# alehdaghi/vq-vae-2-pytorch

Measured on AMD Instinct MI355X. Metric: images/sec VQ-VAE-2 256px train step, higher is better.
Workload: dtype f32; 1 GPU; configs[1]: 256x256 FFHQ-shaped synthetic, default two-level VQ-VAE-2, batch 32/GPU; global_batch=32, image=256, n_embed=512, parallelism=dp1

## Files before the change

include/vq2.h:

```cpp
#ifndef VQ2_H
#define VQ2_H

#include <stddef.h>
#include <stdint.h>

#ifdef __cplusplus
extern "C" {
#endif

#define VQ2_OK 0
#define VQ2_ERR_INVALID 1
#define VQ2_ERR_UNSUPPORTED 2
#define VQ2_ERR_WORKSPACE 3
#define VQ2_ERR_LAUNCH 4

typedef void *vq2_stream_t;

#define VQ2_API_VERSION 6

int vq2_version(void);
const char *vq2_last_error(void);

int vq2_prof_enable(int level);
int vq2_prof_report(char *buf, size_t cap);

typedef struct vq2_conv_desc {
    int32_t N, H, W, Ci;
    int32_t Co;
    int32_t KH, KW, stride, pad;
    int32_t transposed;
    int32_t ldx, ldy;
    int32_t Cir, Cor;
} vq2_conv_desc;

#define VQ2_RELU_IN 1
#define VQ2_RELU_OUT 2

#define VQ2_PACK_FWD 0
#define VQ2_PACK_DGRAD 1
int vq2_pack_weight(const vq2_conv_desc *d, int which, const float *w, float *packed, vq2_stream_t stream);

typedef struct vq2_pack_job {
    const float *w;
    float *packed;
    int64_t offset;
    int64_t numel;
    int32_t Or, Ir, Op, Ip, KH, KW, mode, reserved;
} vq2_pack_job;
int vq2_pack_job_init(const vq2_conv_desc *d, int which, const float *w, float *packed, vq2_pack_job *job);
int vq2_pack_weights_batched(const vq2_pack_job *jobs_dev, int32_t njobs, int64_t total, vq2_stream_t stream);

int vq2_conv_fwd(const vq2_conv_desc *d, int flags, const float *x, const float *wp, const float *bias,
                 const float *residual, int32_t ldres, float *y, vq2_stream_t stream);

int vq2_resblock_supported(int32_t C, int32_t Cm);
int vq2_resblock_fwd(int32_t N, int32_t H, int32_t W, int32_t C, int32_t Cm, int flags, const float *x, int32_t ldx,
                     const float *w1p, const float *b1, const float *w2p, const float *b2, float *r, int32_t ldr,
                     float *y, int32_t ldy, vq2_stream_t stream);

size_t vq2_resblock_w2_workspace_bytes(int32_t N, int32_t H, int32_t W, int32_t C, int32_t Cm);
int vq2_resblock_bwd_data(int32_t N, int32_t H, int32_t W, int32_t C, int32_t Cm, const float *g, int32_t ldg,
                          const float *r, int32_t ldr, const float *x, int32_t ldx, const float *w2d, const float *w1d,
                          float *dh, int32_t lddh, float *dx, int32_t lddx, void *w2_ws, vq2_stream_t stream);

int vq2_conv_dgrad(const vq2_conv_desc *d, const float *dy, const float *wp, const float *mask, int32_t ldmask,
                   const float *residual, int32_t ldres, float *dx, int32_t lddx, vq2_stream_t stream);
#define VQ2_MASK_AFTER_RESIDUAL 4
int vq2_conv_dgrad_ex(const vq2_conv_desc *d, int flags, const float *dy, const float *wp, const float *mask,
                      int32_t ldmask, const float *residual, int32_t ldres, float *dx, int32_t lddx,
                      vq2_stream_t stream);

size_t vq2_conv_wgrad_workspace_bytes(const vq2_conv_desc *d);
int vq2_conv_wgrad(const vq2_conv_desc *d, int flags, const float *x, const float *dy, float *dw, float *db, void *ws,
                   size_t ws_bytes, vq2_stream_t stream);

typedef struct vq2_wgrad_job {
    const float *ws;
    float *dw;
    const float *bias_ws;
    float *db;
    int64_t unit_offset;
    int32_t O, I, Or, Ir, taps, S, n_units_w, n_units_b;
    int32_t swapped;
    int32_t bias_splits;
} vq2_wgrad_job;
int vq2_conv_wgrad_partial(const vq2_conv_desc *d, int flags, const float *x, const float *dy, float *db, void *ws,
                           size_t ws_bytes, vq2_stream_t stream);
int vq2_wgrad_job_init(const vq2_conv_desc *d, const void *ws, float *dw, float *db, vq2_wgrad_job *job);
int vq2_wgrad_reduce_batched(const vq2_wgrad_job *jobs_dev, int32_t njobs, int64_t total_units, vq2_stream_t stream);
int vq2_resblock_w2_job_init(int32_t N, int32_t H, int32_t W, int32_t C, int32_t Cm, const void *ws, float *dw, float *db,
                             vq2_wgrad_job *job);

size_t vq2_colsum_workspace_bytes(int64_t rows, int32_t C);
int vq2_colsum(const float *dy, int64_t rows, int32_t C, int32_t ld, float *db, void *ws, size_t ws_bytes,
               vq2_stream_t stream);

// ... 80 lines not shown
```

vq-vae-2-pytorch_amd/_lib.py:

```python
import ctypes as C
import os

_HERE = os.path.dirname(os.path.abspath(__file__))
LIB_PATH = os.environ.get("VQ2_LIB") or os.path.join(_HERE, "libvq2.so")

c_f32p = C.c_void_p
c_stream = C.c_void_p


class ConvDesc(C.Structure):
    _fields_ = [(n, C.c_int32) for n in
                ("N", "H", "W", "Ci", "Co", "KH", "KW", "stride", "pad", "transposed", "ldx", "ldy", "Cir", "Cor")]


class PackJob(C.Structure):
    _fields_ = [("w", C.c_void_p), ("packed", C.c_void_p), ("offset", C.c_int64), ("numel", C.c_int64)] + \
               [(n, C.c_int32) for n in ("Or", "Ir", "Op", "Ip", "KH", "KW", "mode", "reserved")]


class WgradJob(C.Structure):
    _fields_ = [("ws", C.c_void_p), ("dw", C.c_void_p), ("bias_ws", C.c_void_p), ("db", C.c_void_p),
                ("unit_offset", C.c_int64)] + \
               [(n, C.c_int32) for n in ("O", "I", "Or", "Ir", "taps", "S", "n_units_w", "n_units_b", "swapped", "bias_splits")]

# ... 7 lines not shown
    lib = C.CDLL(LIB_PATH)
    P, I32, I64, SZ, F, D = C.c_void_p, C.c_int32, C.c_int64, C.c_size_t, C.c_float, C.c_double
    DP = C.POINTER(ConvDesc)
    sig = {
        "vq2_version": (C.c_int, []),
        "vq2_last_error": (C.c_char_p, []),
        "vq2_prof_enable": (C.c_int, [C.c_int]),
        "vq2_prof_report": (C.c_int, [C.c_char_p, SZ]),
        "vq2_pack_weight": (C.c_int, [DP, C.c_int, P, P, P]),
        "vq2_pack_job_init": (C.c_int, [DP, C.c_int, P, P, C.POINTER(PackJob)]),
        "vq2_pack_weights_batched": (C.c_int, [P, I32, I64, P]),
        "vq2_conv_fwd": (C.c_int, [DP, C.c_int, P, P, P, P, I32, P, P]),
        "vq2_conv_dgrad": (C.c_int, [DP, P, P, P, I32, P, I32, P, I32, P]),
        "vq2_conv_dgrad_ex": (C.c_int, [DP, C.c_int, P, P, P, I32, P, I32, P, I32, P]),
        "vq2_conv_wgrad_workspace_bytes": (SZ, [DP]),
        "vq2_conv_wgrad": (C.c_int, [DP, C.c_int, P, P, P, P, P, SZ, P]),
        "vq2_conv_wgrad_partial": (C.c_int, [DP, C.c_int, P, P, P, P, SZ, P]),
        "vq2_wgrad_job_init": (C.c_int, [DP, P, P, P, C.POINTER(WgradJob)]),
        "vq2_wgrad_reduce_batched": (C.c_int, [P, I32, I64, P]),
        "vq2_colsum_workspace_bytes": (SZ, [I64, I32]),
        "vq2_colsum": (C.c_int, [P, I64, I32, I32, P, P, SZ, P]),
        "vq2_nchw_to_nhwc": (C.c_int, [P, P, I32, I32, I32, I32, I32, P]),
        "vq2_nhwc_to_nchw": (C.c_int, [P, P, I32, I32, I32, I32, I32, P]),
        "vq2_u8_to_nhwc4": (C.c_int, [P, C.c_int, I32, I32, I32, I32, I32, I32, I32, I32, P, P, P]),
        "vq2_nhwc_to_u8": (C.c_int, [P, I32, I32, I32, I32, I32, C.POINTER(F), C.POINTER(F), P, C.c_int, I32, I32, I64, I32,
                                     I32, I64, P]),
        "vq2_sse_workspace_bytes": (SZ, [I32, I32, I32, I32]),
        "vq2_sse_per_image": (C.c_int, [P, P, I32, I32, I32, I32, P, P, SZ, P]),
        "vq2_index_hist": (C.c_int, [P, I64, I32, P, P, P]),
        "vq2_eval_accumulate": (C.c_int, [P, I32, I64, P, P, P]),
        "vq2_relu_bwd": (C.c_int, [P, I32, P, I32, P, I32, I64, I32, P]),
        "vq2_resblock_supported": (C.c_int, [I32, I32]),
        "vq2_resblock_bwd_data": (C.c_int, [I32, I32, I32, I32, I32, P, I32, P, I32, P, I32, P, P, P, I32, P, I32, P, P]),
        "vq2_resblock_w2_workspace_bytes": (SZ, [I32, I32, I32, I32, I32]),
        "vq2_resblock_w2_job_init": (C.c_int, [I32, I32, I32, I32, I32, P, P, P, C.POINTER(WgradJob)]),
        "vq2_resblock_fwd": (C.c_int, [I32, I32, I32, I32, I32, C.c_int, P, I32, P, P, P, P, P, I32, P, I32, P]),
        "vq2_slice_copy": (C.c_int, [P, I32, P, I32, I64, I32, C.c_int, P]),
        "vq2_vq_prepare": (C.c_int, [P, P, P, I32, I32, P]),
        "vq2_vq_fwd_workspace_floats": (SZ, [I64, I32, I32]),
        "vq2_vq_fwd": (C.c_int, [P, I32, P, P, P, I64, I32, I32, P, P, I32, P, P]),
        "vq2_vq_stats_workspace_bytes": (SZ, [I64, I32, I32]),
        "vq2_vq_stats": (C.c_int, [P, I32, P, I64, I32, I32, P, P, P, SZ, P]),
        "vq2_vq_loss": (C.c_int, [P, I64, I32, P, P]),
        "vq2_vq_bwd": (C.c_int, [P, I32, P, P, I32, P, P, I64, I32, I32, P, I32, P]),
        "vq2_vq_ema_update": (C.c_int, [P, P, P, P, P, I32, I32, D, D, P, P]),
        "vq2_vq_ema_update_prepare": (C.c_int, [P, P, P, P, P, I32, I32, D, D, P, P, P, P]),
        "vq2_vq_gather": (C.c_int, [P, P, I64, I32, I32, P, I32, P]),
        "vq2_instnorm_stats": (C.c_int, [P, I32, I32, I64, I32, D, P, P, P]),
        "vq2_adain_fwd": (C.c_int, [P, I32, P, P, P, I32, I64, I32, C.c_int, P, I32, P]),
        "vq2_adain_bwd": (C.c_int, [P, I32, P, I32, P, I32, P, P, P, I32, I64, I32, P, P, I32, P]),
        "vq2_mse_workspace_bytes": (SZ, [I64]),
        "vq2_mse_fwd_bwd": (C.c_int, [P, P, I64, I64, P, P, P, P, SZ, P]),
        "vq2_stage1_loss": (C.c_int, [P, P, I64, I64, P, F, P, P, P, P, SZ, P]),
        "vq2_adam_step": (C.c_int, [P, P, P, P, I64, D, D, D, D, I32, D, P]),
        "vq2_axpby": (C.c_int, [P, P, F, P, I64, P]),
        "vq2_scale": (C.c_int, [P, P, F, P, I64, P]),
        "vq2_comm_unique_id": (C.c_int, [P]),
        "vq2_comm_init": (C.c_int, [P, I32, I32]),
        "vq2_comm_world": (C.c_int, []),
        "vq2_comm_rank": (C.c_int, []),
        "vq2_comm_allreduce_sum": (C.c_int, [P, I64, P]),
        "vq2_comm_broadcast": (C.c_int, [P, I64, I32, P]),
        "vq2_comm_destroy": (C.c_int, []),
        "vq2_debug_mfma_peak": (C.c_int, [P, I32, I32, P]),
        "vq2_debug_mfma_peak16": (C.c_int, [P, I32, I32, P]),
    }
# ... 26 lines not shown
```

vq-vae-2-pytorch_amd/csrc/vq2_resblock.hip:

```cpp
#include "vq2_common.h"
#include "vq2_rbwino.h"

namespace vq2 {

typedef unsigned int u32x4 __attribute__((ext_vector_type(4)));

namespace rb {
constexpr unsigned RSRC_FLAGS = 0x00020000;
constexpr int OOB = 0x7F000000;
constexpr int TH = 8, TW = 16;
constexpr int PW = TW + 2, PH = TH + 2;
constexpr int NPATCH = PW * PH;
constexpr int CS = 16;
constexpr int LDK = CS + 4;
constexpr int CM = 32;
constexpr int CC = 128;
constexpr int A_F4 = NPATCH * CS / 4;
constexpr int B_F4 = 9 * CM * CS / 4;
constexpr int A_FLOATS = ((A_F4 + 255) / 256) * 64 * LDK;
constexpr int B_FLOATS = ((B_F4 + 255) / 256) * 64 * LDK;
constexpr int LDR = CM + 4;
constexpr size_t LDS_BYTES = (size_t)2 * (A_FLOATS + B_FLOATS) * sizeof(float);
static_assert(2 * LDS_BYTES <= 160 * 1024, "two workgroups per CU");
static_assert(128 * LDR <= 2 * (A_FLOATS + B_FLOATS), "stage-2 aliases fit in the stage-1 buffers");
}

struct ResFwdParams {
    const float *x;
    const float *w1;
    const float *b1;
    const float *w2;
    const float *b2;
    float *r;
    float *y;
// ... 233 lines not shown
        __builtin_amdgcn_raw_buffer_store_b32(__float_as_uint(v), ry, yoff[r] + (NJ - 1) * 128, 0, 0);
    }
}


namespace rbb {
using namespace rb;
constexpr int SA = 32;
constexpr int LDA = SA + 4;
constexpr int PROWS = 192;
constexpr int GA_FLOATS = PROWS * LDA;
constexpr int WA_FLOATS = CM * LDA;
constexpr int WB_FLOATS = CC * LDA;
constexpr size_t LDS_BYTES = (size_t)(2 * GA_FLOATS + 2 * WA_FLOATS) * sizeof(float);
constexpr int WR_FLOATS = 16 * 64 + 32;
constexpr size_t LDS_BYTES_W2 = LDS_BYTES + (size_t)4 * WR_FLOATS * sizeof(float);
static_assert(GA_FLOATS + 2 * WB_FLOATS <= 2 * GA_FLOATS + 2 * WA_FLOATS, "phase-B buffers alias the phase-A ones");
}

struct ResBwdParams {
    const float *g;
    const float *r;
    const float *x;
    const float *w2d;
    const float *w1d;
    float *dh;
    float *dx;
    float *w2_slab;
    float *b2_slab;
    int N, H, W, ldg, ldr, ldx, lddh, lddx;
    int tiles_x, tiles_y;
};

template <bool SAME_LD>
__global__ __launch_bounds__(256, 2) void resblock_bwd_data_kernel(const ResBwdParams P) {
    using namespace rbb;
    extern __shared__ __attribute__((aligned(16))) float smem[];
    float *Ga = smem;
    float *Wa = smem + 2 * GA_FLOATS;
    float *Dh = smem;
    float *Wb = smem + GA_FLOATS;

    const int tid = threadIdx.x, lane = tid & 63, wq = tid >> 6;
    const int l31 = lane & 31, fk = 4 * (lane >> 5), rowq = 4 * (lane >> 5);
    const int tiles = P.tiles_x * P.tiles_y;
    const int vid = xcd_remap(blockIdx.x, gridDim.x);
    const int n = vid / tiles;
    const int t = vid - n * tiles;
    const int tyi = t / P.tiles_x;
    const int y0 = tyi * TH, x0 = (t - tyi * P.tiles_x) * TW;
    const int npix = P.N * P.H * P.W;
    const __amdgpu_buffer_rsrc_t rg = __builtin_amdgcn_make_buffer_rsrc(const_cast<float *>(P.g), 0, npix * P.ldg * 4, RSRC_FLAGS);
    const __amdgpu_buffer_rsrc_t rr = __builtin_amdgcn_make_buffer_rsrc(const_cast<float *>(P.r), 0, npix * P.ldr * 4, RSRC_FLAGS);
    const __amdgpu_buffer_rsrc_t rx = __builtin_amdgcn_make_buffer_rsrc(const_cast<float *>(P.x), 0, npix * P.ldx * 4, RSRC_FLAGS);
    const __amdgpu_buffer_rsrc_t rw2 = __builtin_amdgcn_make_buffer_rsrc(const_cast<float *>(P.w2d), 0, CM * CC * 4, RSRC_FLAGS);
    const __amdgpu_buffer_rsrc_t rw1 = __builtin_amdgcn_make_buffer_rsrc(const_cast<float *>(P.w1d), 0, CC * 9 * CM * 4, RSRC_FLAGS);

    auto patch_pix = [&](int pp) {
        const int pr = pp / PW, pc = pp - pr * PW;
        const int gy = y0 - 1 + pr, gx = x0 - 1 + pc;
        return (pp < NPATCH && (unsigned)gy < (unsigned)P.H && (unsigned)gx < (unsigned)P.W) ? (n * P.H + gy) * P.W + gx : -1;
    };

    constexpr int GA_LD = (NPATCH * (SA / 4) + 255) / 256;
    int ga_off[GA_LD];
#pragma unroll
    for (int j = 0; j < GA_LD; ++j) {
        const int f = tid + 256 * j;
        const int pix = patch_pix(f >> 3);
        ga_off[j] = pix >= 0 ? pix * P.ldg * 4 + (f & 7) * 16 : OOB;
    }
    const int wa_off = ((tid >> 3) * CC) * 4 + (tid & 7) * 16;
    const int st8 = (tid >> 3) * LDA + (tid & 7) * 4;
    constexpr int NSA = CC / SA;
    struct SliceA { u32x4 g[GA_LD], w; };
    auto issue_a = [&](int s, SliceA &r) {
        const int soff = s * SA * 4;
#pragma unroll
        for (int j = 0; j < GA_LD; ++j) r.g[j] = __builtin_amdgcn_raw_buffer_load_b128(rg, ga_off[j], soff, 0);
        r.w = __builtin_amdgcn_raw_buffer_load_b128(rw2, wa_off, soff, 0);
    };
    auto store_a = [&](int s, const SliceA &r) {
        const int buf = s & 1;
        float *a = Ga + buf * GA_FLOATS + st8;
#pragma unroll
        for (int j = 0; j < GA_LD; ++j) *reinterpret_cast<float4 *>(a + j * 32 * LDA) = u4_as_f4(r.g[j]);
        *reinterpret_cast<float4 *>(Wa + buf * WA_FLOATS + st8) = u4_as_f4(r.w);
    };
    static_assert(GA_LD * 256 == PROWS * (SA / 4), "the staging passes cover the padded patch exactly");
    const int nblk = wq < 2 ? 2 : 1;
    SliceA RA0, RA1;
    issue_a(0, RA0);
    issue_a(1, RA1);
    int pixA[2];
    float rmask[2][16];
#pragma unroll
    for (int bi = 0; bi < 2; ++bi) {
        pixA[bi] = patch_pix(32 * (wq + 4 * bi) + l31);
#pragma unroll
        for (int q = 0; q < 16; ++q) {
            const int pix = __shfl(pixA[bi], rowq + (q & 3) + 8 * (q >> 2), 64);
            rmask[bi][q] = __uint_as_float(__builtin_amdgcn_raw_buffer_load_b32(
                rr, (bi < nblk && pix >= 0) ? pix * P.ldr * 4 + l31 * 4 : OOB, 0, 0));
        }
    }
    f32x16 accA[2];
#pragma unroll
    for (int bi = 0; bi < 2; ++bi)
#pragma unroll
        for (int q = 0; q < 16; ++q) accA[bi][q] = 0.f;

    const bool fuse_w2 = P.w2_slab != nullptr;
    float *Wr = smem + 2 * GA_FLOATS + 2 * WA_FLOATS;
    float rB[16];
#pragma unroll
    for (int kk = 0; kk < 16; ++kk) {
        const int q = 2 * kk + (lane >> 5);
        const int gy = y0 + 2 * wq + (q >> 4), gx = x0 + (q & 15);
        const int pix = (gy < P.H && gx < P.W) ? (n * P.H + gy) * P.W + gx : -1;
        rB[kk] = __uint_as_float(__builtin_amdgcn_raw_buffer_load_b32(rr, (fuse_w2 && pix >= 0) ? pix * P.ldr * 4 + l31 * 4 : OOB, 0, 0));
    }
    const int wb_goff = ((tid >> 3) * 9 * CM) * 4 + (tid & 7) * 16;
    u32x4 rwb[4];
    auto issue_b = [&](int tap) {
#pragma unroll
        for (int j = 0; j < 4; ++j) rwb[j] = __builtin_amdgcn_raw_buffer_load_b128(rw1, wb_goff + j * 32 * 9 * CM * 4, tap * CM * 4, 0);
    };
    auto store_b = [&](int buf) {
#pragma unroll
        for (int j = 0; j < 4; ++j) *reinterpret_cast<float4 *>(Wb + buf * WB_FLOATS + st8 + j * 32 * LDA) = u4_as_f4(rwb[j]);
    };

    store_a(0, RA0);
    __syncthreads();
#pragma unroll
    for (int s = 0; s < NSA; ++s) {
        const int buf = s & 1;
        if (s + 1 < NSA) store_a(s + 1, s == 0 ? RA1 : RA0);
        if (s + 2 < NSA) issue_a(s + 2, RA0); else if (s + 2 == NSA) issue_b(0);
        __builtin_amdgcn_sched_barrier(0);
        {
            const float *b = Wa + buf * WA_FLOATS + l31 * LDA + fk;
#pragma unroll
            for (int bi = 0; bi < 2; ++bi) {
                if (bi < nblk) {
                    const float *a = Ga + buf * GA_FLOATS + (32 * (wq + 4 * bi) + l31) * LDA + fk;
#pragma unroll
                    for (int k8 = 0; k8 < SA / 8; ++k8) {
                        const float4 fa = *reinterpret_cast<const float4 *>(a + 8 * k8);
                        const float4 fb = *reinterpret_cast<const float4 *>(b + 8 * k8);
                        accA[bi] = __builtin_amdgcn_mfma_f32_32x32x2f32(fa.x, fb.x, accA[bi], 0, 0, 0);
                        accA[bi] = __builtin_amdgcn_mfma_f32_32x32x2f32(fa.y, fb.y, accA[bi], 0, 0, 0);
                        accA[bi] = __builtin_amdgcn_mfma_f32_32x32x2f32(fa.z, fb.z, accA[bi], 0, 0, 0);
                        accA[bi] = __builtin_amdgcn_mfma_f32_32x32x2f32(fa.w, fb.w, accA[bi], 0, 0, 0);
                    }
                }
            }
        }
        if (fuse_w2) {
            f32x16 aw;
#pragma unroll
            for (int r = 0; r < 16; ++r) aw[r] = 0.f;
            float bs = 0.f;
            const float *ga = Ga + buf * GA_FLOATS + l31;
#pragma unroll
            for (int kk = 0; kk < 16; ++kk) {
                const int q = 2 * kk + (lane >> 5);
                const float a = ga[((2 * wq + (q >> 4) + 1) * PW + (q & 15) + 1) * LDA];
                aw = __builtin_amdgcn_mfma_f32_32x32x2f32(a, rB[kk], aw, 0, 0, 0);
                bs += a;
            }
            float *wr = Wr + wq * WR_FLOATS;
#pragma unroll
            for (int r = 0; r < 16; ++r) wr[r * 64 + lane] = aw[r];
            bs += __shfl_xor(bs, 32, 64);
            if (lane < 32) wr[16 * 64 + lane] = bs;
        }
        __builtin_amdgcn_sched_barrier(0);
        __syncthreads();
        if (fuse_w2) {
            float *slab = P.w2_slab + ((size_t)blockIdx.x * CC + s * 32) * CM;
#pragma unroll
            for (int i = 0; i < 4; ++i) {
                const int r = 4 * wq + i;
                const float v = (Wr[r * 64 + lane] + Wr[WR_FLOATS + r * 64 + lane]) + (Wr[2 * WR_FLOATS + r * 64 + lane] + Wr[3 * WR_FLOATS + r * 64 + lane]);
                slab[(rowq + (r & 3) + 8 * (r >> 2)) * CM + l31] = v;
            }
            if (wq == 0 && lane < 32)
                P.b2_slab[(size_t)blockIdx.x * CC + s * 32 + lane] =
                    (Wr[16 * 64 + lane] + Wr[WR_FLOATS + 16 * 64 + lane]) + (Wr[2 * WR_FLOATS + 16 * 64 + lane] + Wr[3 * WR_FLOATS + 16 * 64 + lane]);
            __syncthreads();
        }
    }
    store_b(0);
    issue_b(1);
    {
        const __amdgpu_buffer_rsrc_t rdh = __builtin_amdgcn_make_buffer_rsrc(P.dh, 0, npix * P.lddh * 4, RSRC_FLAGS);
#pragma unroll
        for (int bi = 0; bi < 2; ++bi) {
            if (bi < nblk) {
                const int pp = 32 * (wq + 4 * bi) + l31;
                const int pr = pp / PW, pc = pp - pr * PW;
                const int own = (pr >= 1 && pr <= TH && pc >= 1 && pc <= TW) ? pixA[bi] : -1;
#pragma unroll
                for (int q = 0; q < 16; ++q) {
                    const int row = rowq + (q & 3) + 8 * (q >> 2);
                    const float v = rmask[bi][q] > 0.f ? accA[bi][q] : 0.f;
                    Dh[(32 * (wq + 4 * bi) + row) * LDA + l31] = v;
                    const int pix = __shfl(own, row, 64);
                    __builtin_amdgcn_raw_buffer_store_b32(__float_as_uint(v), rdh, pix >= 0 ? pix * P.lddh * 4 + l31 * 4 : OOB, 0, 0);
                }
            }
        }
    }
    __syncthreads();

    f32x16 acc[4];
#pragma unroll
    for (int j = 0; j < 4; ++j)
#pragma unroll
        for (int q = 0; q < 16; ++q) acc[j][q] = 0.f;
    const int txr = l31 < 16 ? l31 : ((l31 + 14) & 15);
    const int a_frag = ((2 * wq + (l31 >> 4)) * PW + txr) * LDA + fk;
    int poff[16];
    int pixr[SAME_LD ? 1 : 16];
    {
        const int gy = y0 + 2 * wq + (l31 >> 4), gx = x0 + txr;
        const int pix_lane = (gy < P.H && gx < P.W) ? (n * P.H + gy) * P.W + gx : -1;
#pragma unroll
        for (int q = 0; q < 16; ++q) {
            const int pix = __shfl(pix_lane, rowq + (q & 3) + 8 * (q >> 2), 64);
            poff[q] = pix >= 0 ? pix * (P.ldx * 4) + l31 * 4 : OOB;
            if (!SAME_LD) pixr[q] = pix;
        }
    }
    float mtmp[16], gres[4][16];
    unsigned mbits[2] = {0u, 0u};
    auto issue_b_one = [&](int tap, int j) {
        rwb[j] = __builtin_amdgcn_raw_buffer_load_b128(rw1, wb_goff + j * 32 * 9 * CM * 4, tap * CM * 4, 0);
    };
    auto store_b_one = [&](int buf, int j) {
        *reinterpret_cast<float4 *>(Wb + buf * WB_FLOATS + st8 + j * 32 * LDA) = u4_as_f4(rwb[j]);
    };
#pragma unroll
    for (int tap = 0; tap < 9; ++tap) {
        const int buf = tap & 1;
        __builtin_amdgcn_sched_barrier(0);
        {
            const float *a = Dh + a_frag + ((tap / 3) * PW + (tap % 3)) * LDA;
            const float *b = Wb + buf * WB_FLOATS + l31 * LDA + fk;
            float4 fa[2], fb[2];
            fa[0] = *reinterpret_cast<const float4 *>(a);
            fb[0] = *reinterpret_cast<const float4 *>(b);
#pragma unroll
            for (int g = 0; g < 16; ++g) {
                const int k8 = g >> 2, j = g & 3, cur = g & 1, nxt = cur ^ 1, ca = k8 & 1;
                if (g + 1 < 16) {
                    const int k8n = (g + 1) >> 2, jn = (g + 1) & 3;
                    fb[nxt] = *reinterpret_cast<const float4 *>(b + jn * 32 * LDA + 8 * k8n);
                    if (jn == 0) fa[k8n & 1] = *reinterpret_cast<const float4 *>(a + 8 * k8n);
                }
                acc[j] = __builtin_amdgcn_mfma_f32_32x32x2f32(fa[ca].x, fb[cur].x, acc[j], 0, 0, 0);
                acc[j] = __builtin_amdgcn_mfma_f32_32x32x2f32(fa[ca].y, fb[cur].y, acc[j], 0, 0, 0);
                acc[j] = __builtin_amdgcn_mfma_f32_32x32x2f32(fa[ca].z, fb[cur].z, acc[j], 0, 0, 0);
                acc[j] = __builtin_amdgcn_mfma_f32_32x32x2f32(fa[ca].w, fb[cur].w, acc[j], 0, 0, 0);
                if (g + 1 < 16) {
                    if (((g + 1) & 3) == 0) __builtin_amdgcn_sched_group_barrier(0x100, 2, 0);
                    else __builtin_amdgcn_sched_group_barrier(0x100, 1, 0);
                }
                __builtin_amdgcn_sched_group_barrier(0x008, 4, 0);
                __builtin_amdgcn_sched_barrier(0);
                if (g < 4 && tap + 1 < 9) store_b_one(buf ^ 1, g);
                if (g >= 4 && g < 8 && tap + 2 < 9) issue_b_one(tap + 2, g - 4);
                if (tap < 4 && g < 8) {
#pragma unroll
                    for (int q = 2 * g; q < 2 * g + 2; ++q)
                        mtmp[q] = __uint_as_float(__builtin_amdgcn_raw_buffer_load_b32(rx, poff[q], tap * 128, 0));
                }
                if (tap >= 5)
                    gres[tap - 5][g] = __uint_as_float(__builtin_amdgcn_raw_buffer_load_b32(
                        rg, SAME_LD ? poff[g] : (pixr[SAME_LD ? 0 : g] >= 0 ? pixr[SAME_LD ? 0 : g] * P.ldg * 4 + l31 * 4 : OOB),
                        (tap - 5) * 128, 0));
                __builtin_amdgcn_sched_barrier(0);
            }
        }
        __builtin_amdgcn_sched_barrier(0);
        if (tap < 4) {
#pragma unroll
            for (int q = 0; q < 16; ++q) mbits[tap >> 1] |= (mtmp[q] > 0.f ? 1u : 0u) << ((tap & 1) * 16 + q);
        }
        __syncthreads();
    }
    const __amdgpu_buffer_rsrc_t rdx = __builtin_amdgcn_make_buffer_rsrc(P.dx, 0, npix * P.lddx * 4, RSRC_FLAGS);
#pragma unroll
    for (int j = 0; j < 4; ++j)
#pragma unroll
        for (int q = 0; q < 16; ++q) {
            float v = ((mbits[j >> 1] >> ((j & 1) * 16 + q)) & 1u) ? acc[j][q] : 0.f;
            v += gres[j][q];
            __builtin_amdgcn_raw_buffer_store_b32(
                __float_as_uint(v), rdx,
                SAME_LD ? poff[q] : (pixr[SAME_LD ? 0 : q] >= 0 ? pixr[SAME_LD ? 0 : q] * P.lddx * 4 + l31 * 4 : OOB), j * 128, 0);
        }
}

}

extern "C" int vq2_resblock_supported(int32_t C, int32_t Cm) { return (C == vq2::rb::CC && Cm == vq2::rb::CM) ? 1 : 0; }

extern "C" int vq2_resblock_fwd(int32_t N, int32_t H, int32_t W, int32_t C, int32_t Cm, int flags, const float *x,
                                int32_t ldx, const float *w1p, const float *b1, const float *w2p, const float *b2,
                                float *r, int32_t ldr, float *y, int32_t ldy, vq2_stream_t stream) {
    using namespace vq2;
    VQ2_REQUIRE(N > 0 && H > 0 && W > 0, "resblock_fwd: empty tensor");
    if (int e = check_forms()) return e;
    if (!vq2_resblock_supported(C, Cm))
        return set_error(VQ2_ERR_UNSUPPORTED, "resblock_fwd: fused kernel is built for channel=%d, n_res_channel=%d (got %d, %d)",
                         rb::CC, rb::CM, C, Cm);
    VQ2_REQUIRE(x && w1p && b1 && w2p && b2 && r && y, "resblock_fwd: null pointer");
    VQ2_REQUIRE(aligned16(x) && aligned16(w1p) && aligned16(w2p) && aligned16(r) && aligned16(y),
                "resblock_fwd: pointers must be 16-byte aligned");
    VQ2_REQUIRE(ldx >= C && ldy >= C && ldr >= Cm && ldx % 4 == 0 && ldy % 4 == 0 && ldr % 4 == 0,
                "resblock_fwd: pixel strides must cover the channels and be multiples of 4");
    VQ2_REQUIRE((flags & ~VQ2_RELU_OUT) == 0, "resblock_fwd: only VQ2_RELU_OUT is a valid flag");
    const double npix = (double)N * H * W;
    const int ldmax = ldx > ldy ? ldx : ldy;
    VQ2_REQUIRE(npix * ldmax * 4.0 < (double)rb::OOB, "resblock_fwd: tensors must be smaller than %d bytes", rb::OOB);
    {
        RbwFwdParams Q{};
        Q.x = x; Q.w1 = w1p; Q.b1 = b1; Q.w2 = w2p; Q.b2 = b2; Q.r = r; Q.y = y;
        Q.N = N; Q.H = H; Q.W = W; Q.ldx = ldx; Q.ldr = ldr; Q.ldy = ldy; Q.relu_out = (flags & VQ2_RELU_OUT) != 0;
        if (ldr >= Cm && rbw_fwd_ok(Q)) {
            hipStream_t s = to_stream(stream);
            const char *name = "resblock_fwd_wino";
            if (prof_enabled()) name = prof_label("resblock_fwd_wino|M=%d,C=%d,Cm=%d", N * H * W, C, Cm);
// ... 10 lines not shown
    hipStream_t s = to_stream(stream);
    const char *name = "resblock_fwd";
    if (prof_enabled()) name = prof_label("resblock_fwd|M=%d,C=%d,Cm=%d", N * H * W, C, Cm);
    ProfScope prof(name, 2.0 * npix * (9.0 * C * Cm + (double)Cm * C), 4.0 * npix * (2.0 * C + Cm), s);
    allow_big_lds(resblock_fwd_kernel, rb::LDS_BYTES);
    hipLaunchKernelGGL(resblock_fwd_kernel, dim3(grid), dim3(256), rb::LDS_BYTES, s, P);
    return check_launch("resblock_fwd_kernel");
}

static int rb_grid(int N, int H, int W) { return N * ((W + vq2::rb::TW - 1) / vq2::rb::TW) * ((H + vq2::rb::TH - 1) / vq2::rb::TH); }

extern "C" size_t vq2_resblock_w2_workspace_bytes(int32_t N, int32_t H, int32_t W, int32_t C, int32_t Cm) {
    if (N <= 0 || H <= 0 || W <= 0 || !vq2_resblock_supported(C, Cm)) return 0;
    return (size_t)rb_grid(N, H, W) * ((size_t)C * Cm + C) * sizeof(float);
}

extern "C" int vq2_resblock_w2_job_init(int32_t N, int32_t H, int32_t W, int32_t C, int32_t Cm, const void *ws, float *dw,
                                        float *db, vq2_wgrad_job *job) {
    VQ2_REQUIRE(ws && dw && job && vq2_resblock_supported(C, Cm) && N > 0 && H > 0 && W > 0, "resblock_w2_job_init: bad arguments");
    const int S = rb_grid(N, H, W);
    const float *w = static_cast<const float *>(ws);
    job->ws = w; job->dw = dw; job->bias_ws = db ? w + (size_t)S * C * Cm : nullptr; job->db = db;
    job->unit_offset = 0;
    job->O = C; job->I = Cm; job->Or = C; job->Ir = Cm; job->taps = 1; job->S = S;
    job->n_units_w = (C * Cm + 31) / 32; job->n_units_b = db ? (C + 31) / 32 : 0;
    job->swapped = 0; job->bias_splits = 0;
    return VQ2_OK;
}

extern "C" int vq2_resblock_bwd_data(int32_t N, int32_t H, int32_t W, int32_t C, int32_t Cm, const float *g, int32_t ldg,
                                     const float *r, int32_t ldr, const float *x, int32_t ldx, const float *w2d,
                                     const float *w1d, float *dh, int32_t lddh, float *dx, int32_t lddx, void *w2_ws,
                                     vq2_stream_t stream) {
    using namespace vq2;
    VQ2_REQUIRE(N > 0 && H > 0 && W > 0, "resblock_bwd_data: empty tensor");
    if (!vq2_resblock_supported(C, Cm))
        return set_error(VQ2_ERR_UNSUPPORTED, "resblock_bwd_data: fused kernel is built for channel=%d, n_res_channel=%d (got %d, %d)",
                         rb::CC, rb::CM, C, Cm);
    VQ2_REQUIRE(g && r && x && w2d && w1d && dh && dx, "resblock_bwd_data: null pointer");
    VQ2_REQUIRE(aligned16(g) && aligned16(r) && aligned16(x) && aligned16(w2d) && aligned16(w1d) && aligned16(dh) && aligned16(dx),
                "resblock_bwd_data: pointers must be 16-byte aligned");
    VQ2_REQUIRE(ldg >= C && ldx >= C && lddx >= C && ldr >= Cm && lddh >= Cm && ldg % 4 == 0 && ldx % 4 == 0 &&
                    lddx % 4 == 0 && ldr % 4 == 0 && lddh % 4 == 0,
                "resblock_bwd_data: pixel strides must cover the channels and be multiples of 4");
    const double npix = (double)N * H * W;
    int ldmax = ldg > ldx ? ldg : ldx;
    if (lddx > ldmax) ldmax = lddx;
    VQ2_REQUIRE(npix * ldmax * 4.0 < (double)rb::OOB, "resblock_bwd_data: tensors must be smaller than %d bytes", rb::OOB);
    ResBwdParams P{};
    P.g = g; P.r = r; P.x = x; P.w2d = w2d; P.w1d = w1d; P.dh = dh; P.dx = dx;
    VQ2_REQUIRE(!w2_ws || aligned16(w2_ws), "resblock_bwd_data: workspace must be 16-byte aligned");
    P.N = N; P.H = H; P.W = W; P.ldg = ldg; P.ldr = ldr; P.ldx = ldx; P.lddh = lddh; P.lddx = lddx;
    P.tiles_x = (W + rb::TW - 1) / rb::TW; P.tiles_y = (H + rb::TH - 1) / rb::TH;
    const int grid = N * P.tiles_x * P.tiles_y;
    hipStream_t s = to_stream(stream);
    const char *name = "resblock_bwd_data";
    if (prof_enabled()) name = prof_label("resblock_bwd_data|M=%d,C=%d,Cm=%d", N * H * W, C, Cm);
    ProfScope prof(name, 2.0 * npix * (9.0 * C * Cm + (double)Cm * C), 4.0 * npix * (4.0 * C + 2.0 * Cm), s);
    P.w2_slab = static_cast<float *>(w2_ws);
    P.b2_slab = w2_ws ? P.w2_slab + (size_t)grid * C * Cm : nullptr;
    const size_t lds = w2_ws ? rbb::LDS_BYTES_W2 : rbb::LDS_BYTES;
    if (ldg == ldx && lddx == ldx) {
        allow_big_lds(resblock_bwd_data_kernel<true>, lds);
        hipLaunchKernelGGL(resblock_bwd_data_kernel<true>, dim3(grid), dim3(256), lds, s, P);
    } else {
        allow_big_lds(resblock_bwd_data_kernel<false>, lds);
        hipLaunchKernelGGL(resblock_bwd_data_kernel<false>, dim3(grid), dim3(256), lds, s, P);
    }
    return check_launch("resblock_bwd_data_kernel");
}
```

vq-vae-2-pytorch_amd/ops.py:

```python
from dataclasses import dataclass
import ctypes as C
import os

import torch
from torch.autograd import Function

from ._lib import lib, check, ConvDesc, PackJob, WgradJob

VQ2_RELU_IN = 1
VQ2_RELU_OUT = 2
VQ2_MASK_AFTER_RESIDUAL = 4
PACK_FWD = 0
PACK_DGRAD = 1



def _stream():
    return C.c_void_p(torch.cuda.current_stream().cuda_stream)


def _p(t):
    return None if t is None else C.c_void_p(t.data_ptr())


# ... 576 lines not shown
        if out is not None:
            y = y.view_as(y)
        return y

    @staticmethod
    def backward(ctx, dy):
        x, r, w1, w2, y, b1, b2 = ctx.saved_tensors
        s1, s2 = ctx.spec1, ctx.spec2
        g = as_nhwc(dy)
        if ctx.relu_out and not ctx.premasked:
            g = relu_bwd(g, y)
        n, h, w, c = x.shape
        if RESBLOCK_FUSED[0] and ctx.needs_input_grad[0] and lib.vq2_resblock_supported(c, s1.co) and s1.k == 3 and s2.k == 1:
            dh = torch.empty((n, h, w, s1.co), device=x.device, dtype=torch.float32)
            dx = torch.empty((n, h, w, c), device=x.device, dtype=torch.float32)
            sc = _step_ctx(w2)
            w2_ws = None
            if (sc is not None and ctx.needs_input_grad[3] and ctx.needs_input_grad[4] and
                    getattr(w2, "_vq2_grad", None) is not None and getattr(b2, "_vq2_grad", None) is not None and
                    w2.grad is None and b2.grad is None):
                w2_ws, dw2, db2 = sc.batch.resblock_w2(n, h, w, c, s1.co, w2, b2)
            check(lib.vq2_resblock_bwd_data(n, h, w, c, s1.co, _p(g), ld_of(g), _p(r), ld_of(r), _p(x), ld_of(x),
                                            _p(packed_weight(s2, w2, PACK_DGRAD)), _p(packed_weight(s1, w1, PACK_DGRAD)),
                                            _p(dh), ld_of(dh), _p(dx), ld_of(dx), _p(w2_ws), _stream()), "resblock_bwd_data")
            if w2_ws is not None:
                dw1, db1 = conv_wgrad(s1, x, dh, True, w1, b1, ctx.needs_input_grad[1], ctx.needs_input_grad[2])
                return dx, dw1, db1, dw2, db2, None, None, None, None, None
        else:
            dh = conv_dgrad(s2, r.shape, g, w2, mask=r)
            dx = conv_dgrad(s1, x.shape, dh, w1, mask=x, residual=g) if ctx.needs_input_grad[0] else None
        dw2, db2 = conv_wgrad(s2, r, g, False, w2, b2, ctx.needs_input_grad[3], ctx.needs_input_grad[4])
        dw1, db1 = conv_wgrad(s1, x, dh, True, w1, b1, ctx.needs_input_grad[1], ctx.needs_input_grad[2])
        return dx, dw1, db1, dw2, db2, None, None, None, None, None


class CatViewFn(Function):

    @staticmethod
    def forward(ctx, a, b, buf, stash=None):
        ctx.ca = a.shape[3]
        ctx.stash = stash
        return buf.view_as(buf)

    @staticmethod
    def backward(ctx, g):
        g = as_nhwc(g)
        gb = g[..., ctx.ca:]
        if ctx.stash is not None:
            if ctx.stash.put(gb):
                gb = None
            elif ctx.stash.strict:
                raise RuntimeError("GradStash: the consumer that applies b's ReLU mask ran before this gradient arrived")
        return g[..., :ctx.ca], gb, None, None


class CatFn(Function):

    @staticmethod
    def forward(ctx, a, b):
        a, b = as_nhwc(a), as_nhwc(b)
        n, h, w, ca = a.shape
        cb = b.shape[3]
        if tuple(b.shape[:3]) != (n, h, w):
            raise RuntimeError("CatFn: spatial sizes differ")
        out = torch.empty((n, h, w, ca + cb), device=a.device, dtype=torch.float32)
        pix = n * h * w
# ... 275 lines not shown
```

Measured before the change: 5465 images/s.

## Add eight-wave variant of fused resblock backward kernel for small feature maps

Templates the fused resblock backward-data kernel on wave count and adds an eight-wave (512-thread) form. It is picked automatically when W <= 32, and callers can also request it explicitly. In the eight-wave form the output channel blocks are split across two wave groups, and only half the waves compute the fused w2 weight gradient. The goal is more parallelism per block on small feature maps, where the grid has few tiles and the GPU is underfilled. The cost is lower occupancy per CU (launch bounds drop to 1 block) and narrower staging loads.

```diff
diff --git a/include/vq2.h b/include/vq2.h
--- a/include/vq2.h
+++ b/include/vq2.h
@@ -16,7 +16,7 @@
 
 typedef void *vq2_stream_t;
 
-#define VQ2_API_VERSION 6
+#define VQ2_API_VERSION 7
 
 int vq2_version(void);
 const char *vq2_last_error(void);
@@ -62,6 +62,13 @@
 int vq2_resblock_bwd_data(int32_t N, int32_t H, int32_t W, int32_t C, int32_t Cm, const float *g, int32_t ldg,
                           const float *r, int32_t ldr, const float *x, int32_t ldx, const float *w2d, const float *w1d,
                           float *dh, int32_t lddh, float *dx, int32_t lddx, void *w2_ws, vq2_stream_t stream);
+#define VQ2_RB_BWD_BY_SHAPE 0
+#define VQ2_RB_BWD_WAVES4 1
+#define VQ2_RB_BWD_WAVES8 2
+int vq2_resblock_bwd_data_form(int32_t N, int32_t H, int32_t W, int32_t C, int32_t Cm, const float *g, int32_t ldg,
+                               const float *r, int32_t ldr, const float *x, int32_t ldx, const float *w2d,
+                               const float *w1d, float *dh, int32_t lddh, float *dx, int32_t lddx, void *w2_ws, int form,
+                               vq2_stream_t stream);
 
 int vq2_conv_dgrad(const vq2_conv_desc *d, const float *dy, const float *wp, const float *mask, int32_t ldmask,
                    const float *residual, int32_t ldres, float *dx, int32_t lddx, vq2_stream_t stream);
diff --git a/vq-vae-2-pytorch_amd/_lib.py b/vq-vae-2-pytorch_amd/_lib.py
--- a/vq-vae-2-pytorch_amd/_lib.py
+++ b/vq-vae-2-pytorch_amd/_lib.py
@@ -63,6 +63,7 @@
         "vq2_relu_bwd": (C.c_int, [P, I32, P, I32, P, I32, I64, I32, P]),
         "vq2_resblock_supported": (C.c_int, [I32, I32]),
         "vq2_resblock_bwd_data": (C.c_int, [I32, I32, I32, I32, I32, P, I32, P, I32, P, I32, P, P, P, I32, P, I32, P, P]),
+        "vq2_resblock_bwd_data_form": (C.c_int, [I32, I32, I32, I32, I32, P, I32, P, I32, P, I32, P, P, P, I32, P, I32, P, C.c_int, P]),
         "vq2_resblock_w2_workspace_bytes": (SZ, [I32, I32, I32, I32, I32]),
         "vq2_resblock_w2_job_init": (C.c_int, [I32, I32, I32, I32, I32, P, P, P, C.POINTER(WgradJob)]),
         "vq2_resblock_fwd": (C.c_int, [I32, I32, I32, I32, I32, C.c_int, P, I32, P, P, P, P, P, I32, P, I32, P]),
diff --git a/vq-vae-2-pytorch_amd/csrc/vq2_resblock.hip b/vq-vae-2-pytorch_amd/csrc/vq2_resblock.hip
--- a/vq-vae-2-pytorch_amd/csrc/vq2_resblock.hip
+++ b/vq-vae-2-pytorch_amd/csrc/vq2_resblock.hip
@@ -1,5 +1,6 @@
 #include "vq2_common.h"
 #include "vq2_rbwino.h"
+#include <type_traits>
 
 namespace vq2 {
 
@@ -299,9 +300,14 @@
     int tiles_x, tiles_y;
 };
 
-template <bool SAME_LD>
-__global__ __launch_bounds__(256, 2) void resblock_bwd_data_kernel(const ResBwdParams P) {
+template <bool SAME_LD, int NW>
+__global__ __launch_bounds__(NW * 64, NW == 4 ? 2 : 1) void resblock_bwd_data_kernel(const ResBwdParams P) {
     using namespace rbb;
+    static_assert(NW == 4 || NW == 8, "four or eight waves");
+    constexpr int NT = NW * 64;
+    constexpr int SROWS = NT / 8;
+    constexpr int ABLK = NW == 4 ? 2 : 1;
+    constexpr int NJ = 16 / NW;
     extern __shared__ __attribute__((aligned(16))) float smem[];
     float *Ga = smem;
     float *Wa = smem + 2 * GA_FLOATS;
@@ -310,6 +316,8 @@
 
     const int tid = threadIdx.x, lane = tid & 63, wq = tid >> 6;
     const int l31 = lane & 31, fk = 4 * (lane >> 5), rowq = 4 * (lane >> 5);
+    const int pb = NW == 4 ? wq : (wq & 3);
+    const int cb0 = NW == 4 ? 0 : 2 * (wq >> 2);
     const int tiles = P.tiles_x * P.tiles_y;
     const int vid = xcd_remap(blockIdx.x, gridDim.x);
     const int n = vid / tiles;
@@ -329,40 +337,46 @@
         return (pp < NPATCH && (unsigned)gy < (unsigned)P.H && (unsigned)gx < (unsigned)P.W) ? (n * P.H + gy) * P.W + gx : -1;
     };
 
-    constexpr int GA_LD = (NPATCH * (SA / 4) + 255) / 256;
+    constexpr int GA_LD = (NPATCH * (SA / 4) + NT - 1) / NT;
     int ga_off[GA_LD];
 #pragma unroll
     for (int j = 0; j < GA_LD; ++j) {
-        const int f = tid + 256 * j;
+        const int f = tid + NT * j;
         const int pix = patch_pix(f >> 3);
         ga_off[j] = pix >= 0 ? pix * P.ldg * 4 + (f & 7) * 16 : OOB;
     }
-    const int wa_off = ((tid >> 3) * CC) * 4 + (tid & 7) * 16;
+    typedef unsigned int u32x2 __attribute__((ext_vector_type(2)));
+    using WaVec = std::conditional_t<NW == 4, u32x4, u32x2>;
+    const int wa_off = NW == 4 ? ((tid >> 3) * CC) * 4 + (tid & 7) * 16 : ((tid >> 4) * CC) * 4 + (tid & 15) * 8;
+    const int wa_st = NW == 4 ? (tid >> 3) * LDA + (tid & 7) * 4 : (tid >> 4) * LDA + (tid & 15) * 2;
     const int st8 = (tid >> 3) * LDA + (tid & 7) * 4;
     constexpr int NSA = CC / SA;
-    struct SliceA { u32x4 g[GA_LD], w; };
+    struct SliceA { u32x4 g[GA_LD]; WaVec w; };
     auto issue_a = [&](int s, SliceA &r) {
         const int soff = s * SA * 4;
 #pragma unroll
         for (int j = 0; j < GA_LD; ++j) r.g[j] = __builtin_amdgcn_raw_buffer_load_b128(rg, ga_off[j], soff, 0);
-        r.w = __builtin_amdgcn_raw_buffer_load_b128(rw2, wa_off, soff, 0);
+        if constexpr (NW == 4) r.w = __builtin_amdgcn_raw_buffer_load_b128(rw2, wa_off, soff, 0);
+        else r.w = __builtin_amdgcn_raw_buffer_load_b64(rw2, wa_off, soff, 0);
     };
     auto store_a = [&](int s, const SliceA &r) {
         const int buf = s & 1;
         float *a = Ga + buf * GA_FLOATS + st8;
 #pragma unroll
-        for (int j = 0; j < GA_LD; ++j) *reinterpret_cast<float4 *>(a + j * 32 * LDA) = u4_as_f4(r.g[j]);
-        *reinterpret_cast<float4 *>(Wa + buf * WA_FLOATS + st8) = u4_as_f4(r.w);
-    };
-    static_assert(GA_LD * 256 == PROWS * (SA / 4), "the staging passes cover the padded patch exactly");
-    const int nblk = wq < 2 ? 2 : 1;
+        for (int j = 0; j < GA_LD; ++j) *reinterpret_cast<float4 *>(a + j * SROWS * LDA) = u4_as_f4(r.g[j]);
+        if constexpr (NW == 4) *reinterpret_cast<float4 *>(Wa + buf * WA_FLOATS + wa_st) = u4_as_f4(r.w);
+        else *reinterpret_cast<float2 *>(Wa + buf * WA_FLOATS + wa_st) = make_float2(__uint_as_float(r.w.x), __uint_as_float(r.w.y));
+    };
+    static_assert(GA_LD * NT == PROWS * (SA / 4), "the staging passes cover the padded patch exactly");
+    static_assert(NT * (NW == 4 ? 4 : 2) == CM * SA, "the panel slice is one vector per thread");
+    const int nblk = NW == 4 ? (wq < 2 ? 2 : 1) : (wq < 6 ? 1 : 0);
     SliceA RA0, RA1;
     issue_a(0, RA0);
     issue_a(1, RA1);
-    int pixA[2];
-    float rmask[2][16];
-#pragma unroll
-    for (int bi = 0; bi < 2; ++bi) {
+    int pixA[ABLK];
+    float rmask[ABLK][16];
+#pragma unroll
+    for (int bi = 0; bi < ABLK; ++bi) {
         pixA[bi] = patch_pix(32 * (wq + 4 * bi) + l31);
 #pragma unroll
         for (int q = 0; q < 16; ++q) {
@@ -371,31 +385,34 @@
                 rr, (bi < nblk && pix >= 0) ? pix * P.ldr * 4 + l31 * 4 : OOB, 0, 0));
         }
     }
-    f32x16 accA[2];
-#pragma unroll
-    for (int bi = 0; bi < 2; ++bi)
+    f32x16 accA[ABLK];
+#pragma unroll
+    for (int bi = 0; bi < ABLK; ++bi)
 #pragma unroll
         for (int q = 0; q < 16; ++q) accA[bi][q] = 0.f;
 
     const bool fuse_w2 = P.w2_slab != nullptr;
+    const bool w2_wave = NW == 4 || wq >= 4;
     float *Wr = smem + 2 * GA_FLOATS + 2 * WA_FLOATS;
     float rB[16];
 #pragma unroll
     for (int kk = 0; kk < 16; ++kk) {
         const int q = 2 * kk + (lane >> 5);
-        const int gy = y0 + 2 * wq + (q >> 4), gx = x0 + (q & 15);
+        const int gy = y0 + 2 * pb + (q >> 4), gx = x0 + (q & 15);
         const int pix = (gy < P.H && gx < P.W) ? (n * P.H + gy) * P.W + gx : -1;
-        rB[kk] = __uint_as_float(__builtin_amdgcn_raw_buffer_load_b32(rr, (fuse_w2 && pix >= 0) ? pix * P.ldr * 4 + l31 * 4 : OOB, 0, 0));
+        rB[kk] = __uint_as_float(__builtin_amdgcn_raw_buffer_load_b32(rr, (fuse_w2 && w2_wave && pix >= 0) ? pix * P.ldr * 4 + l31 * 4 : OOB, 0, 0));
     }
     const int wb_goff = ((tid >> 3) * 9 * CM) * 4 + (tid & 7) * 16;
-    u32x4 rwb[4];
+    constexpr int WB_LD = CC * (CM / 4) / NT;
+    static_assert(WB_LD * SROWS == CC, "the staging passes cover the tap panel exactly");
+    u32x4 rwb[WB_LD];
     auto issue_b = [&](int tap) {
 #pragma unroll
-        for (int j = 0; j < 4; ++j) rwb[j] = __builtin_amdgcn_raw_buffer_load_b128(rw1, wb_goff + j * 32 * 9 * CM * 4, tap * CM * 4, 0);
+        for (int j = 0; j < WB_LD; ++j) rwb[j] = __builtin_amdgcn_raw_buffer_load_b128(rw1, wb_goff + j * SROWS * 9 * CM * 4, tap * CM * 4, 0);
     };
     auto store_b = [&](int buf) {
 #pragma unroll
-        for (int j = 0; j < 4; ++j) *reinterpret_cast<float4 *>(Wb + buf * WB_FLOATS + st8 + j * 32 * LDA) = u4_as_f4(rwb[j]);
+        for (int j = 0; j < WB_LD; ++j) *reinterpret_cast<float4 *>(Wb + buf * WB_FLOATS + st8 + j * SROWS * LDA) = u4_as_f4(rwb[j]);
     };
 
     store_a(0, RA0);
@@ -409,7 +426,7 @@
         {
             const float *b = Wa + buf * WA_FLOATS + l31 * LDA + fk;
 #pragma unroll
-            for (int bi = 0; bi < 2; ++bi) {
+            for (int bi = 0; bi < ABLK; ++bi) {
                 if (bi < nblk) {
                     const float *a = Ga + buf * GA_FLOATS + (32 * (wq + 4 * bi) + l31) * LDA + fk;
 #pragma unroll
@@ -424,7 +441,7 @@
                 }
             }
         }
-        if (fuse_w2) {
+        if (fuse_w2 && w2_wave) {
             f32x16 aw;
 #pragma unroll
             for (int r = 0; r < 16; ++r) aw[r] = 0.f;
@@ -433,11 +450,11 @@
 #pragma unroll
             for (int kk = 0; kk < 16; ++kk) {
                 const int q = 2 * kk + (lane >> 5);
-                const float a = ga[((2 * wq + (q >> 4) + 1) * PW + (q & 15) + 1) * LDA];
+                const float a = ga[((2 * pb + (q >> 4) + 1) * PW + (q & 15) + 1) * LDA];
                 aw = __builtin_amdgcn_mfma_f32_32x32x2f32(a, rB[kk], aw, 0, 0, 0);
                 bs += a;
             }
-            float *wr = Wr + wq * WR_FLOATS;
+            float *wr = Wr + pb * WR_FLOATS;
 #pragma unroll
             for (int r = 0; r < 16; ++r) wr[r * 64 + lane] = aw[r];
             bs += __shfl_xor(bs, 32, 64);
@@ -448,8 +465,8 @@
         if (fuse_w2) {
             float *slab = P.w2_slab + ((size_t)blockIdx.x * CC + s * 32) * CM;
 #pragma unroll
-            for (int i = 0; i < 4; ++i) {
-                const int r = 4 * wq + i;
+            for (int i = 0; i < NJ; ++i) {
+                const int r = NJ * wq + i;
                 const float v = (Wr[r * 64 + lane] + Wr[WR_FLOATS + r * 64 + lane]) + (Wr[2 * WR_FLOATS + r * 64 + lane] + Wr[3 * WR_FLOATS + r * 64 + lane]);
                 slab[(rowq + (r & 3) + 8 * (r >> 2)) * CM + l31] = v;
             }
@@ -464,7 +481,7 @@
     {
         const __amdgpu_buffer_rsrc_t rdh = __builtin_amdgcn_make_buffer_rsrc(P.dh, 0, npix * P.lddh * 4, RSRC_FLAGS);
 #pragma unroll
-        for (int bi = 0; bi < 2; ++bi) {
+        for (int bi = 0; bi < ABLK; ++bi) {
             if (bi < nblk) {
                 const int pp = 32 * (wq + 4 * bi) + l31;
                 const int pr = pp / PW, pc = pp - pr * PW;
@@ -482,48 +499,50 @@
     }
     __syncthreads();
 
-    f32x16 acc[4];
-#pragma unroll
-    for (int j = 0; j < 4; ++j)
+    f32x16 acc[NJ];
+#pragma unroll
+    for (int j = 0; j < NJ; ++j)
 #pragma unroll
         for (int q = 0; q < 16; ++q) acc[j][q] = 0.f;
     const int txr = l31 < 16 ? l31 : ((l31 + 14) & 15);
-    const int a_frag = ((2 * wq + (l31 >> 4)) * PW + txr) * LDA + fk;
+    const int a_frag = ((2 * pb + (l31 >> 4)) * PW + txr) * LDA + fk;
     int poff[16];
     int pixr[SAME_LD ? 1 : 16];
     {
-        const int gy = y0 + 2 * wq + (l31 >> 4), gx = x0 + txr;
+        const int gy = y0 + 2 * pb + (l31 >> 4), gx = x0 + txr;
         const int pix_lane = (gy < P.H && gx < P.W) ? (n * P.H + gy) * P.W + gx : -1;
 #pragma unroll
         for (int q = 0; q < 16; ++q) {
             const int pix = __shfl(pix_lane, rowq + (q & 3) + 8 * (q >> 2), 64);
-            poff[q] = pix >= 0 ? pix * (P.ldx * 4) + l31 * 4 : OOB;
+            poff[q] = pix >= 0 ? pix * (P.ldx * 4) + (cb0 * 32 + l31) * 4 : OOB;
             if (!SAME_LD) pixr[q] = pix;
         }
     }
-    float mtmp[16], gres[4][16];
-    unsigned mbits[2] = {0u, 0u};
+    float mtmp[16], gres[NJ][16];
+    unsigned mbits[(NJ + 1) / 2] = {};
     auto issue_b_one = [&](int tap, int j) {
-        rwb[j] = __builtin_amdgcn_raw_buffer_load_b128(rw1, wb_goff + j * 32 * 9 * CM * 4, tap * CM * 4, 0);
+        rwb[j] = __builtin_amdgcn_raw_buffer_load_b128(rw1, wb_goff + j * SROWS * 9 * CM * 4, tap * CM * 4, 0);
     };
     auto store_b_one = [&](int buf, int j) {
-        *reinterpret_cast<float4 *>(Wb + buf * WB_FLOATS + st8 + j * 32 * LDA) = u4_as_f4(rwb[j]);
-    };
+        *reinterpret_cast<float4 *>(Wb + buf * WB_FLOATS + st8 + j * SROWS * LDA) = u4_as_f4(rwb[j]);
+    };
+    constexpr int NG = 4 * NJ;
+    constexpr int ML = 16 / (NG / 2);
 #pragma unroll
     for (int tap = 0; tap < 9; ++tap) {
         const int buf = tap & 1;
         __builtin_amdgcn_sched_barrier(0);
         {
             const float *a = Dh + a_frag + ((tap / 3) * PW + (tap % 3)) * LDA;
-            const float *b = Wb + buf * WB_FLOATS + l31 * LDA + fk;
+            const float *b = Wb + buf * WB_FLOATS + (cb0 * 32 + l31) * LDA + fk;
             float4 fa[2], fb[2];
             fa[0] = *reinterpret_cast<const float4 *>(a);
             fb[0] = *reinterpret_cast<const float4 *>(b);
 #pragma unroll
-            for (int g = 0; g < 16; ++g) {
-                const int k8 = g >> 2, j = g & 3, cur = g & 1, nxt = cur ^ 1, ca = k8 & 1;
-                if (g + 1 < 16) {
-                    const int k8n = (g + 1) >> 2, jn = (g + 1) & 3;
+            for (int g = 0; g < NG; ++g) {
+                const int k8 = g / NJ, j = g % NJ, cur = g & 1, nxt = cur ^ 1, ca = k8 & 1;
+                if (g + 1 < NG) {
+                    const int k8n = (g + 1) / NJ, jn = (g + 1) % NJ;
                     fb[nxt] = *reinterpret_cast<const float4 *>(b + jn * 32 * LDA + 8 * k8n);
                     if (jn == 0) fa[k8n & 1] = *reinterpret_cast<const float4 *>(a + 8 * k8n);
                 }
@@ -531,28 +550,30 @@
                 acc[j] = __builtin_amdgcn_mfma_f32_32x32x2f32(fa[ca].y, fb[cur].y, acc[j], 0, 0, 0);
                 acc[j] = __builtin_amdgcn_mfma_f32_32x32x2f32(fa[ca].z, fb[cur].z, acc[j], 0, 0, 0);
                 acc[j] = __builtin_amdgcn_mfma_f32_32x32x2f32(fa[ca].w, fb[cur].w, acc[j], 0, 0, 0);
-                if (g + 1 < 16) {
-                    if (((g + 1) & 3) == 0) __builtin_amdgcn_sched_group_barrier(0x100, 2, 0);
+                if (g + 1 < NG) {
+                    if (((g + 1) % NJ) == 0) __builtin_amdgcn_sched_group_barrier(0x100, 2, 0);
                     else __builtin_amdgcn_sched_group_barrier(0x100, 1, 0);
                 }
                 __builtin_amdgcn_sched_group_barrier(0x008, 4, 0);
                 __builtin_amdgcn_sched_barrier(0);
-                if (g < 4 && tap + 1 < 9) store_b_one(buf ^ 1, g);
-                if (g >= 4 && g < 8 && tap + 2 < 9) issue_b_one(tap + 2, g - 4);
-                if (tap < 4 && g < 8) {
-#pragma unroll
-                    for (int q = 2 * g; q < 2 * g + 2; ++q)
+                if (g < WB_LD && tap + 1 < 9) store_b_one(buf ^ 1, g);
+                if (g >= WB_LD && g < 2 * WB_LD && tap + 2 < 9) issue_b_one(tap + 2, g - WB_LD);
+                if (tap < NJ && g < NG / 2) {
+#pragma unroll
+                    for (int q = ML * g; q < ML * g + ML; ++q)
                         mtmp[q] = __uint_as_float(__builtin_amdgcn_raw_buffer_load_b32(rx, poff[q], tap * 128, 0));
                 }
-                if (tap >= 5)
-                    gres[tap - 5][g] = __uint_as_float(__builtin_amdgcn_raw_buffer_load_b32(
-                        rg, SAME_LD ? poff[g] : (pixr[SAME_LD ? 0 : g] >= 0 ? pixr[SAME_LD ? 0 : g] * P.ldg * 4 + l31 * 4 : OOB),
-                        (tap - 5) * 128, 0));
+                if (tap >= 5) {
+                    const int gi = (tap - 5) * NG + g, gj = gi / 16, gq = gi % 16;
+                    gres[gj][gq] = __uint_as_float(__builtin_amdgcn_raw_buffer_load_b32(
+                        rg, SAME_LD ? poff[gq] : (pixr[SAME_LD ? 0 : gq] >= 0 ? pixr[SAME_LD ? 0 : gq] * P.ldg * 4 + (cb0 * 32 + l31) * 4 : OOB),
+                        gj * 128, 0));
+                }
                 __builtin_amdgcn_sched_barrier(0);
             }
         }
         __builtin_amdgcn_sched_barrier(0);
-        if (tap < 4) {
+        if (tap < NJ) {
 #pragma unroll
             for (int q = 0; q < 16; ++q) mbits[tap >> 1] |= (mtmp[q] > 0.f ? 1u : 0u) << ((tap & 1) * 16 + q);
         }
@@ -560,14 +581,14 @@
     }
     const __amdgpu_buffer_rsrc_t rdx = __builtin_amdgcn_make_buffer_rsrc(P.dx, 0, npix * P.lddx * 4, RSRC_FLAGS);
 #pragma unroll
-    for (int j = 0; j < 4; ++j)
+    for (int j = 0; j < NJ; ++j)
 #pragma unroll
         for (int q = 0; q < 16; ++q) {
             float v = ((mbits[j >> 1] >> ((j & 1) * 16 + q)) & 1u) ? acc[j][q] : 0.f;
             v += gres[j][q];
             __builtin_amdgcn_raw_buffer_store_b32(
                 __float_as_uint(v), rdx,
-                SAME_LD ? poff[q] : (pixr[SAME_LD ? 0 : q] >= 0 ? pixr[SAME_LD ? 0 : q] * P.lddx * 4 + l31 * 4 : OOB), j * 128, 0);
+                SAME_LD ? poff[q] : (pixr[SAME_LD ? 0 : q] >= 0 ? pixr[SAME_LD ? 0 : q] * P.lddx * 4 + (cb0 * 32 + l31) * 4 : OOB), j * 128, 0);
         }
 }
 
@@ -644,7 +665,23 @@
                                      const float *r, int32_t ldr, const float *x, int32_t ldx, const float *w2d,
                                      const float *w1d, float *dh, int32_t lddh, float *dx, int32_t lddx, void *w2_ws,
                                      vq2_stream_t stream) {
+    return vq2_resblock_bwd_data_form(N, H, W, C, Cm, g, ldg, r, ldr, x, ldx, w2d, w1d, dh, lddh, dx, lddx, w2_ws,
+                                      VQ2_RB_BWD_BY_SHAPE, stream);
+}
+
+template <bool SAME_LD, int NW>
+static void launch_rb_bwd(const vq2::ResBwdParams &P, int grid, size_t lds, hipStream_t s) {
+    vq2::allow_big_lds(vq2::resblock_bwd_data_kernel<SAME_LD, NW>, lds);
+    hipLaunchKernelGGL((vq2::resblock_bwd_data_kernel<SAME_LD, NW>), dim3(grid), dim3(NW * 64), lds, s, P);
+}
+
+extern "C" int vq2_resblock_bwd_data_form(int32_t N, int32_t H, int32_t W, int32_t C, int32_t Cm, const float *g, int32_t ldg,
+                                          const float *r, int32_t ldr, const float *x, int32_t ldx, const float *w2d,
+                                          const float *w1d, float *dh, int32_t lddh, float *dx, int32_t lddx, void *w2_ws,
+                                          int form, vq2_stream_t stream) {
     using namespace vq2;
+    VQ2_REQUIRE(form == VQ2_RB_BWD_BY_SHAPE || form == VQ2_RB_BWD_WAVES4 || form == VQ2_RB_BWD_WAVES8,
+                "resblock_bwd_data: form must be VQ2_RB_BWD_BY_SHAPE, _WAVES4 or _WAVES8");
     VQ2_REQUIRE(N > 0 && H > 0 && W > 0, "resblock_bwd_data: empty tensor");
     if (!vq2_resblock_supported(C, Cm))
         return set_error(VQ2_ERR_UNSUPPORTED, "resblock_bwd_data: fused kernel is built for channel=%d, n_res_channel=%d (got %d, %d)",
@@ -666,18 +703,18 @@
     P.tiles_x = (W + rb::TW - 1) / rb::TW; P.tiles_y = (H + rb::TH - 1) / rb::TH;
     const int grid = N * P.tiles_x * P.tiles_y;
     hipStream_t s = to_stream(stream);
+    const bool wide = form == VQ2_RB_BWD_BY_SHAPE ? W <= 32 : form == VQ2_RB_BWD_WAVES8;
     const char *name = "resblock_bwd_data";
-    if (prof_enabled()) name = prof_label("resblock_bwd_data|M=%d,C=%d,Cm=%d", N * H * W, C, Cm);
+    if (prof_enabled()) name = prof_label("resblock_bwd_data|M=%d,C=%d,Cm=%d,%s", N * H * W, C, Cm, wide ? "w8" : "w4");
     ProfScope prof(name, 2.0 * npix * (9.0 * C * Cm + (double)Cm * C), 4.0 * npix * (4.0 * C + 2.0 * Cm), s);
     P.w2_slab = static_cast<float *>(w2_ws);
     P.b2_slab = w2_ws ? P.w2_slab + (size_t)grid * C * Cm : nullptr;
     const size_t lds = w2_ws ? rbb::LDS_BYTES_W2 : rbb::LDS_BYTES;
-    if (ldg == ldx && lddx == ldx) {
-        allow_big_lds(resblock_bwd_data_kernel<true>, lds);
-        hipLaunchKernelGGL(resblock_bwd_data_kernel<true>, dim3(grid), dim3(256), lds, s, P);
+    const bool same_ld = ldg == ldx && lddx == ldx;
+    if (wide) {
+        if (same_ld) launch_rb_bwd<true, 8>(P, grid, lds, s); else launch_rb_bwd<false, 8>(P, grid, lds, s);
     } else {
-        allow_big_lds(resblock_bwd_data_kernel<false>, lds);
-        hipLaunchKernelGGL(resblock_bwd_data_kernel<false>, dim3(grid), dim3(256), lds, s, P);
+        if (same_ld) launch_rb_bwd<true, 4>(P, grid, lds, s); else launch_rb_bwd<false, 4>(P, grid, lds, s);
     }
     return check_launch("resblock_bwd_data_kernel");
 }
diff --git a/vq-vae-2-pytorch_amd/ops.py b/vq-vae-2-pytorch_amd/ops.py
--- a/vq-vae-2-pytorch_amd/ops.py
+++ b/vq-vae-2-pytorch_amd/ops.py
@@ -632,6 +632,20 @@
         dw2, db2 = conv_wgrad(s2, r, g, False, w2, b2, ctx.needs_input_grad[3], ctx.needs_input_grad[4])
         dw1, db1 = conv_wgrad(s1, x, dh, True, w1, b1, ctx.needs_input_grad[1], ctx.needs_input_grad[2])
         return dx, dw1, db1, dw2, db2, None, None, None, None, None
+
+
+RB_BWD_BY_SHAPE, RB_BWD_WAVES4, RB_BWD_WAVES8 = 0, 1, 2
+
+
+def resblock_bwd_data_form(g, r, x, w2d, w1d, form=RB_BWD_BY_SHAPE, w2_ws=None):
+    n, h, w, c = x.shape
+    cm = r.shape[3]
+    dh = torch.empty((n, h, w, cm), device=x.device, dtype=torch.float32)
+    dx = torch.empty((n, h, w, c), device=x.device, dtype=torch.float32)
+    check(lib.vq2_resblock_bwd_data_form(n, h, w, c, cm, _p(g), ld_of(g), _p(r), ld_of(r), _p(x), ld_of(x), _p(w2d), _p(w1d),
+                                         _p(dh), ld_of(dh), _p(dx), ld_of(dx), _p(w2_ws), form, _stream()),
+          "resblock_bwd_data_form")
+    return dh, dx
 
 
 class CatViewFn(Function):
```

After: 5477 images/s, median of 6. About the same (+0.2%).
